# sudhirverma/distributed-ranges

Measured on AMD Instinct MI355X. Metric: elements/s & % HBM roofline: reduce/scan/sort/SpMV at 1/2/4/8 MI355X, higher is better.
Workload: dtype f32

## Files before the change

### distributed-ranges_amd/include/dr/shp/merge_sort.hpp

```cpp
#pragma once

#include <hip/hip_runtime.h>

#include <algorithm>
#include <cstddef>
#include <cstdint>

namespace shp::detail::msort {

constexpr int kMsBlock = 256;
template <typename T> constexpr int ipt() {
  return sizeof(T) <= 4 ? 8 : sizeof(T) <= 8 ? 8 : sizeof(T) <= 16 ? 4 : sizeof(T) <= 32 ? 2 : 1;
}
template <typename T> constexpr int pad_every() { return ipt<T>() >= 4 ? ipt<T>() : 0; }
template <typename T> constexpr std::size_t padded(std::size_t e) {
  return pad_every<T>() ? e + e / pad_every<T>() : e;
}
#ifndef DR_SHP_MSORT_SORT_THREADS
#define DR_SHP_MSORT_SORT_THREADS 256
#endif
static_assert(DR_SHP_MSORT_SORT_THREADS >= kMsBlock && (DR_SHP_MSORT_SORT_THREADS & (DR_SHP_MSORT_SORT_THREADS - 1)) == 0,
              "DR_SHP_MSORT_SORT_THREADS must be a power of two and at least kMsBlock");
template <typename T> constexpr int sort_threads() {
  return padded<T>(std::size_t(DR_SHP_MSORT_SORT_THREADS) * ipt<T>()) * sizeof(T) <= 65536 ? DR_SHP_MSORT_SORT_THREADS
                                                                                         : kMsBlock;
}
template <typename T> constexpr std::size_t tile() { return std::size_t(kMsBlock) * ipt<T>(); }
template <typename T> constexpr std::size_t sort_tile() { return std::size_t(sort_threads<T>()) * ipt<T>(); }

template <typename I, typename PA, typename PB, typename Comp>
__host__ __device__ inline I merge_path(PA a, I na, PB b, I nb, I diag, Comp &comp) {
  I lo = diag > nb ? diag - nb : 0, hi = diag < na ? diag : na;
  while (lo < hi) {
    const I mid = (lo + hi) / 2;
    if (!comp(b[diag - 1 - mid], a[mid])) lo = mid + 1;
    else hi = mid;
  }
  return lo;
}

template <typename T> struct lds_view {
  T *s;
  int off;
  __device__ T &operator[](int i) const {
    const int j = off + i;
    return s[pad_every<T>() ? j + j / pad_every<T>() : j];
  }
  __device__ lds_view at(int o) const { return {s, off + o}; }
};

template <int N, typename T, typename Comp>
__device__ inline int serial_merge(lds_view<T> v, int ai, int aend, int bi, int bend, T (&y)[N], Comp &comp) {
  int cnt = 0;
#pragma unroll
  for (int k = 0; k < N; k++) {
    if (ai < aend || bi < bend) {
      const bool take_b = bi < bend && (ai >= aend || comp(v[bi], v[ai]));
      if (take_b) y[k] = v[bi++];
      else y[k] = v[ai++];
      cnt = k + 1;
    }
  }
  return cnt;
}

template <typename T, std::size_t E> struct lds_tile {
  alignas(alignof(T) > 16 ? alignof(T) : 16) unsigned char raw[padded<T>(E) * sizeof(T)];
  __device__ lds_view<T> view() { return {reinterpret_cast<T *>(raw), 0}; }
};

template <typename T, typename Comp>
__global__ __launch_bounds__(sort_threads<T>()) void block_sort_kernel(T *data, std::size_t n, Comp comp) {
  constexpr int NT = sort_threads<T>();
  constexpr int N = ipt<T>();
  constexpr int TILE = (int)sort_tile<T>();
  __shared__ lds_tile<T, sort_tile<T>()> lds;
  const lds_view<T> s = lds.view();
  const std::size_t base = (std::size_t)blockIdx.x * TILE;
  const int cnt = (int)std::min<std::size_t>(TILE, n - base);
  {
    T r[N];
#pragma unroll
    for (int k = 0; k < N; k++)
      if (k * NT + (int)threadIdx.x < cnt) r[k] = data[base + k * NT + threadIdx.x];
#pragma unroll
    for (int k = 0; k < N; k++)
      if (k * NT + (int)threadIdx.x < cnt) s[k * NT + threadIdx.x] = r[k];
  }
  __syncthreads();
  const int my = threadIdx.x * N;
  const int valid = std::max(0, std::min(N, cnt - my));
  T x[N];
#pragma unroll
  for (int k = 0; k < N; k++)
    if (k < valid) x[k] = s[my + k];
#pragma unroll
  for (int r = 0; r < N; r++) {
#pragma unroll
    for (int k = r & 1; k + 1 < N; k += 2)
      if (k + 1 < valid && comp(x[k + 1], x[k])) {
        const T t = x[k];
        x[k] = x[k + 1];
        x[k + 1] = t;
      }
  }
  __syncthreads();
#pragma unroll
  for (int k = 0; k < N; k++)
    if (k < valid) s[my + k] = x[k];
  __syncthreads();
  for (int coop = 2; coop <= NT; coop *= 2) {
    const int lane = threadIdx.x % coop;
    const int g0 = (threadIdx.x / coop) * coop * N, half = coop / 2 * N;
    const int a0 = std::min(g0, cnt), a1 = std::min(g0 + half, cnt), b1 = std::min(g0 + 2 * half, cnt);
    const int na = a1 - a0, nb = b1 - a1;
    const int diag = std::min(lane * N, na + nb);
    const int i = merge_path<int>(s.at(a0), na, s.at(a1), nb, diag, comp);
    T y[N];
    const int got = serial_merge<N>(s, a0 + i, a1, a1 + diag - i, b1, y, comp);
    __syncthreads();
#pragma unroll
    for (int k = 0; k < N; k++)
      if (k < got) s[a0 + diag + k] = y[k];
    __syncthreads();
  }
#pragma unroll
  for (int k = 0; k < N; k++)
    if (k * NT + (int)threadIdx.x < cnt) data[base + k * NT + threadIdx.x] = s[k * NT + threadIdx.x];
}

struct pass_geom {
  std::size_t n, w;
  bool single;
  __host__ __device__ std::size_t pair_base(std::size_t d) const { return single ? 0 : d / (2 * w) * (2 * w); }
  __host__ __device__ std::size_t pair_end(std::size_t pb) const { return single ? n : std::min(n, pb + 2 * w); }
  __host__ __device__ std::size_t na(std::size_t pb) const { return std::min(w, n - pb); }
};

template <typename T, typename Comp>
__global__ void merge_partition_kernel(const T *src, pass_geom g, std::size_t ntiles, std::size_t *part, Comp comp) {
  const std::size_t t = (std::size_t)blockIdx.x * blockDim.x + threadIdx.x;
  if (t >= ntiles) return;
  const std::size_t d = t * tile<T>();
  const std::size_t pb = g.pair_base(d), na = g.na(pb), nb = g.pair_end(pb) - pb - na;
  part[t] = merge_path<std::size_t>(src + pb, na, src + pb + na, nb, d - pb, comp);
}

template <typename T, typename Comp>
__global__ __launch_bounds__(kMsBlock) void merge_kernel(const T *src, T *dst, pass_geom g, std::size_t ntiles,
                                                         const std::size_t *part, Comp comp) {
  constexpr int N = ipt<T>();
  constexpr std::size_t TILE = tile<T>();
  __shared__ lds_tile<T, tile<T>()> lds;
  const lds_view<T> s = lds.view();
  const std::size_t t = blockIdx.x;
  const std::size_t d0 = t * TILE, pb = g.pair_base(d0), pe = g.pair_end(pb);
  const std::size_t d1 = std::min(d0 + TILE, pe);
  const std::size_t na = g.na(pb);
  const std::size_t i0 = part[t];
  const std::size_t i1 = (t + 1 < ntiles && (t + 1) * TILE < pe) ? part[t + 1] : na;
  const std::size_t j0 = (d0 - pb) - i0, j1 = (d1 - pb) - i1;
  const T *A = src + pb, *B = src + pb + na;
  const int la = (int)(i1 - i0), lb = (int)(j1 - j0);
  {
    T r[N];
#pragma unroll
    for (int k = 0; k < N; k++) {
      const int e = k * kMsBlock + threadIdx.x;
      if (e < la) r[k] = A[i0 + e];
      else if (e < la + lb) r[k] = B[j0 + (e - la)];
    }
#pragma unroll
    for (int k = 0; k < N; k++) {
      const int e = k * kMsBlock + threadIdx.x;
      if (e < la + lb) s[e] = r[k];
    }
  }
  __syncthreads();
  const int diag = std::min((int)threadIdx.x * N, la + lb);
  const int i = merge_path<int>(s, la, s.at(la), lb, diag, comp);
  T y[N];
  const int got = serial_merge<N>(s, i, la, la + diag - i, la + lb, y, comp);
  __syncthreads();
#pragma unroll
  for (int k = 0; k < N; k++)
    if (k < got) s[diag + k] = y[k];
  __syncthreads();
#pragma unroll
  for (int k = 0; k < N; k++)
    if (k * kMsBlock + (int)threadIdx.x < la + lb) dst[d0 + k * kMsBlock + threadIdx.x] = s[k * kMsBlock + threadIdx.x];
}

template <typename T> __global__ void gather_samples_kernel(const T *data, std::size_t stride, std::size_t ns, T *s) {
  const std::size_t j = (std::size_t)blockIdx.x * blockDim.x + threadIdx.x;
  if (j < ns) s[j] = data[j * stride];
}

template <typename T> constexpr std::size_t scratch_bytes(std::size_t n) {
  const std::size_t tiles = (n + tile<T>() - 1) / tile<T>();
  return ((n * sizeof(T) + 255) & ~std::size_t(255)) + (tiles + 1) * sizeof(std::size_t);
}

inline unsigned blocks_of(std::size_t n, std::size_t per) { return (unsigned)std::max<std::size_t>(1, (n + per - 1) / per); }

template <typename T, typename Comp>
void merge_pass(const T *src, T *dst, pass_geom g, std::size_t *part, Comp comp, hipStream_t st) {
  const std::size_t ntiles = (g.n + tile<T>() - 1) / tile<T>();
  hipLaunchKernelGGL((merge_partition_kernel<T, Comp>), dim3(blocks_of(ntiles, 256)), dim3(256), 0, st, src, g,
                     ntiles, part, comp);
  hipLaunchKernelGGL((merge_kernel<T, Comp>), dim3((unsigned)ntiles), dim3(kMsBlock), 0, st, src, dst, g, ntiles,
                     part, comp);
}

template <typename T, typename Comp>
void local_sort(T *data, std::size_t n, void *scratch, Comp comp, hipStream_t st) {
  if (n <= 1) return;
  T *tmp = static_cast<T *>(scratch);
  auto *part = reinterpret_cast<std::size_t *>(static_cast<char *>(scratch) + ((n * sizeof(T) + 255) & ~std::size_t(255)));
  hipLaunchKernelGGL((block_sort_kernel<T, Comp>), dim3(blocks_of(n, sort_tile<T>())), dim3(sort_threads<T>()), 0,
                     st, data, n, comp);
  T *src = data, *dst = tmp;
  for (std::size_t w = sort_tile<T>(); w < n; w *= 2) {
    merge_pass<T>(src, dst, pass_geom{n, w, false}, part, comp, st);
    std::swap(src, dst);
  }
  if (src != data) (void)hipMemcpyAsync(data, src, n * sizeof(T), hipMemcpyDeviceToDevice, st);
}

}
```

Measured before the change: 533.2 billion.

## Vectorize merge-sort loads/stores, enlarge block-sort tile, remove final copy via parity

For 2/4-byte types, the block sort and merge kernels now stage global data into LDS with 16-byte vector loads. The final merge step writes each thread's outputs straight to global memory, skipping the LDS round trip and the last barriers. The block-sort tile doubles items per thread, which cuts one merge pass. The starting buffer is chosen by pass parity so the sorted result lands in `data`, removing the trailing device copy. The cost is register pressure from 16 items per thread, and direct per-thread output stores may coalesce less well than the old strided writes.

```diff
diff --git a/distributed-ranges_amd/include/dr/shp/merge_sort.hpp b/distributed-ranges_amd/include/dr/shp/merge_sort.hpp
--- a/distributed-ranges_amd/include/dr/shp/merge_sort.hpp
+++ b/distributed-ranges_amd/include/dr/shp/merge_sort.hpp
@@ -16,17 +16,14 @@
 template <typename T> constexpr std::size_t padded(std::size_t e) {
   return pad_every<T>() ? e + e / pad_every<T>() : e;
 }
-#ifndef DR_SHP_MSORT_SORT_THREADS
-#define DR_SHP_MSORT_SORT_THREADS 256
-#endif
-static_assert(DR_SHP_MSORT_SORT_THREADS >= kMsBlock && (DR_SHP_MSORT_SORT_THREADS & (DR_SHP_MSORT_SORT_THREADS - 1)) == 0,
-              "DR_SHP_MSORT_SORT_THREADS must be a power of two and at least kMsBlock");
-template <typename T> constexpr int sort_threads() {
-  return padded<T>(std::size_t(DR_SHP_MSORT_SORT_THREADS) * ipt<T>()) * sizeof(T) <= 65536 ? DR_SHP_MSORT_SORT_THREADS
-                                                                                         : kMsBlock;
-}
+template <typename T> constexpr int sort_threads() { return kMsBlock; }
+template <typename T> constexpr int sort_ipt() { return sizeof(T) <= 8 ? 2 * ipt<T>() : ipt<T>(); }
 template <typename T> constexpr std::size_t tile() { return std::size_t(kMsBlock) * ipt<T>(); }
-template <typename T> constexpr std::size_t sort_tile() { return std::size_t(sort_threads<T>()) * ipt<T>(); }
+template <typename T> constexpr std::size_t sort_tile() { return std::size_t(sort_threads<T>()) * sort_ipt<T>(); }
+template <typename T> constexpr bool sort_tile_ok() {
+  return sort_tile<T>() % tile<T>() == 0 && (sort_threads<T>() & (sort_threads<T>() - 1)) == 0 &&
+         padded<T>(sort_tile<T>()) * sizeof(T) <= 65536;
+}
 
 template <typename I, typename PA, typename PB, typename Comp>
 __host__ __device__ inline I merge_path(PA a, I na, PB b, I nb, I diag, Comp &comp) {
@@ -39,6 +36,25 @@
   return lo;
 }
 
+template <typename T> constexpr bool wide_type() { return sizeof(T) == 2 || sizeof(T) == 4; }
+template <typename T> constexpr int vec_elems() { return 16 % sizeof(T) == 0 ? 16 / (int)sizeof(T) : 1; }
+struct alignas(16) vec16 {
+  std::uint32_t w[4];
+};
+
+struct wide_ranges {
+  int head, nvec, tail;
+};
+template <typename T> __host__ __device__ inline wide_ranges wide_split(std::uintptr_t addr, int len) {
+  constexpr int V = vec_elems<T>();
+  const int mis = (int)(addr & 15);
+  if (16 % sizeof(T) != 0 || mis % (int)sizeof(T)) return {len, 0, 0};
+  const int to_boundary = ((16 - mis) & 15) / (int)sizeof(T);
+  const int head = len < to_boundary ? len : to_boundary;
+  const int nvec = (len - head) / V;
+  return {head, nvec, len - head - nvec * V};
+}
+
 template <typename T> struct lds_view {
   T *s;
   int off;
@@ -69,20 +85,78 @@
   __device__ lds_view<T> view() { return {reinterpret_cast<T *>(raw), 0}; }
 };
 
-template <typename T, typename Comp>
-__global__ __launch_bounds__(sort_threads<T>()) void block_sort_kernel(T *data, std::size_t n, Comp comp) {
+template <int NT, int NI, typename T> struct wide_piece {
+  static constexpr int V = vec_elems<T>();
+  static constexpr int NVT = NI / V > 0 ? NI / V : 1;
+  vec16 r[NVT];
+  wide_ranges g;
+  __device__ void load(const T *p, int len) {
+    g = wide_split<T>(reinterpret_cast<std::uintptr_t>(p), len);
+    const vec16 *pv = reinterpret_cast<const vec16 *>(p + g.head);
+#pragma unroll
+    for (int k = 0; k < NVT; k++)
+      if (k * NT + (int)threadIdx.x < g.nvec) r[k] = pv[k * NT + threadIdx.x];
+  }
+  __device__ void store(const T *p, lds_view<T> s) const {
+    const int body = g.head + g.nvec * V;
+    for (int e = threadIdx.x; e < g.head + g.tail; e += NT) {
+      const int i = e < g.head ? e : body + (e - g.head);
+      s[i] = p[i];
+    }
+#pragma unroll
+    for (int k = 0; k < NVT; k++)
+      if (k * NT + (int)threadIdx.x < g.nvec) {
+        T e[V];
+        __builtin_memcpy(e, &r[k], 16);
+#pragma unroll
+        for (int j = 0; j < V; j++) s[g.head + (k * NT + (int)threadIdx.x) * V + j] = e[j];
+      }
+  }
+};
+
+template <int N, typename T> __device__ inline void store_outputs(T *dst, const T (&y)[N], int got) {
+  static_assert(N * sizeof(T) % 16 == 0, "a thread's outputs are whole 16-byte vectors");
+  if (got == N) {
+    vec16 v[N * sizeof(T) / 16];
+    __builtin_memcpy(v, y, sizeof(v));
+#pragma unroll
+    for (int q = 0; q < (int)(N * sizeof(T) / 16); q++) reinterpret_cast<vec16 *>(dst)[q] = v[q];
+  } else {
+#pragma unroll
+    for (int k = 0; k < N; k++)
+      if (k < got) dst[k] = y[k];
+  }
+}
+
+template <typename T> __device__ inline bool aligned16(const T *a, const T *b) {
+  return ((reinterpret_cast<std::uintptr_t>(a) | reinterpret_cast<std::uintptr_t>(b)) & 15) == 0;
+}
+
+template <typename T, typename Comp>
+__global__ __launch_bounds__(sort_threads<T>()) void block_sort_kernel(const T *src, T *dst, std::size_t n, Comp comp) {
+  static_assert(sort_tile_ok<T>(), "the block sort's tile must be a power-of-two multiple of tile<T>() that fits LDS");
   constexpr int NT = sort_threads<T>();
-  constexpr int N = ipt<T>();
+  constexpr int N = sort_ipt<T>();
   constexpr int TILE = (int)sort_tile<T>();
   __shared__ lds_tile<T, sort_tile<T>()> lds;
   const lds_view<T> s = lds.view();
   const std::size_t base = (std::size_t)blockIdx.x * TILE;
   const int cnt = (int)std::min<std::size_t>(TILE, n - base);
-  {
+  const bool wide = wide_type<T>() && aligned16(src, dst);
+  bool staged = false;
+  if constexpr (wide_type<T>()) {
+    if (wide) {
+      wide_piece<NT, N, T> p;
+      p.load(src + base, cnt);
+      p.store(src + base, s);
+      staged = true;
+    }
+  }
+  if (!staged) {
     T r[N];
 #pragma unroll
     for (int k = 0; k < N; k++)
-      if (k * NT + (int)threadIdx.x < cnt) r[k] = data[base + k * NT + threadIdx.x];
+      if (k * NT + (int)threadIdx.x < cnt) r[k] = src[base + k * NT + threadIdx.x];
 #pragma unroll
     for (int k = 0; k < N; k++)
       if (k * NT + (int)threadIdx.x < cnt) s[k * NT + threadIdx.x] = r[k];
@@ -118,6 +192,12 @@
     const int i = merge_path<int>(s.at(a0), na, s.at(a1), nb, diag, comp);
     T y[N];
     const int got = serial_merge<N>(s, a0 + i, a1, a1 + diag - i, b1, y, comp);
+    if constexpr (wide_type<T>()) {
+      if (wide && coop == NT) {
+        store_outputs<N>(dst + base + diag, y, got);
+        return;
+      }
+    }
     __syncthreads();
 #pragma unroll
     for (int k = 0; k < N; k++)
@@ -126,7 +206,7 @@
   }
 #pragma unroll
   for (int k = 0; k < N; k++)
-    if (k * NT + (int)threadIdx.x < cnt) data[base + k * NT + threadIdx.x] = s[k * NT + threadIdx.x];
+    if (k * NT + (int)threadIdx.x < cnt) dst[base + k * NT + threadIdx.x] = s[k * NT + threadIdx.x];
 }
 
 struct pass_geom {
@@ -162,7 +242,19 @@
   const std::size_t j0 = (d0 - pb) - i0, j1 = (d1 - pb) - i1;
   const T *A = src + pb, *B = src + pb + na;
   const int la = (int)(i1 - i0), lb = (int)(j1 - j0);
-  {
+  const bool wide = wide_type<T>() && aligned16(src, dst);
+  bool staged = false;
+  if constexpr (wide_type<T>()) {
+    if (wide) {
+      wide_piece<kMsBlock, N, T> pa, pb2;
+      pa.load(A + i0, la);
+      pb2.load(B + j0, lb);
+      pa.store(A + i0, s);
+      pb2.store(B + j0, s.at(la));
+      staged = true;
+    }
+  }
+  if (!staged) {
     T r[N];
 #pragma unroll
     for (int k = 0; k < N; k++) {
@@ -181,6 +273,12 @@
   const int i = merge_path<int>(s, la, s.at(la), lb, diag, comp);
   T y[N];
   const int got = serial_merge<N>(s, i, la, la + diag - i, la + lb, y, comp);
+  if constexpr (wide_type<T>()) {
+    if (wide) {
+      store_outputs<N>(dst + d0 + diag, y, got);
+      return;
+    }
+  }
   __syncthreads();
 #pragma unroll
   for (int k = 0; k < N; k++)
@@ -204,10 +302,16 @@
 inline unsigned blocks_of(std::size_t n, std::size_t per) { return (unsigned)std::max<std::size_t>(1, (n + per - 1) / per); }
 
 template <typename T, typename Comp>
-void merge_pass(const T *src, T *dst, pass_geom g, std::size_t *part, Comp comp, hipStream_t st) {
+void merge_partition(const T *src, pass_geom g, std::size_t *part, Comp comp, hipStream_t st) {
   const std::size_t ntiles = (g.n + tile<T>() - 1) / tile<T>();
   hipLaunchKernelGGL((merge_partition_kernel<T, Comp>), dim3(blocks_of(ntiles, 256)), dim3(256), 0, st, src, g,
                      ntiles, part, comp);
+}
+
+template <typename T, typename Comp>
+void merge_pass(const T *src, T *dst, pass_geom g, std::size_t *part, Comp comp, hipStream_t st) {
+  const std::size_t ntiles = (g.n + tile<T>() - 1) / tile<T>();
+  merge_partition<T>(src, g, part, comp, st);
   hipLaunchKernelGGL((merge_kernel<T, Comp>), dim3((unsigned)ntiles), dim3(kMsBlock), 0, st, src, dst, g, ntiles,
                      part, comp);
 }
@@ -217,14 +321,15 @@
   if (n <= 1) return;
   T *tmp = static_cast<T *>(scratch);
   auto *part = reinterpret_cast<std::size_t *>(static_cast<char *>(scratch) + ((n * sizeof(T) + 255) & ~std::size_t(255)));
+  int passes = 0;
+  for (std::size_t w = sort_tile<T>(); w < n; w *= 2) passes++;
+  T *src = passes % 2 ? tmp : data, *dst = src == data ? tmp : data;
   hipLaunchKernelGGL((block_sort_kernel<T, Comp>), dim3(blocks_of(n, sort_tile<T>())), dim3(sort_threads<T>()), 0,
-                     st, data, n, comp);
-  T *src = data, *dst = tmp;
+                     st, data, src, n, comp);
   for (std::size_t w = sort_tile<T>(); w < n; w *= 2) {
     merge_pass<T>(src, dst, pass_geom{n, w, false}, part, comp, st);
     std::swap(src, dst);
   }
-  if (src != data) (void)hipMemcpyAsync(data, src, n * sizeof(T), hipMemcpyDeviceToDevice, st);
-}
-
-}
+}
+
+}
```

Result: no change. 533.2 billion, median of 3 (-0.0%).
